# rubengooj/pl-slam

Hardware: AMD Instinct MI355X
Metric: stereo pairs/sec (1500 ORB + 200 LBD BF-match) (higher is better)
Workload: dtype fp4; 1 GPU; C2: synthetic 752x480 stereo stream, 1500 ORB + 200 LBD per image, ORB+LBD L<->R and prev<->curr, mutual + ratio (StVO::match), then StereoFrame's gates over the L<->R tables (config_kitti.yaml:25-...; mutual=True, distinct_batches_in_rotation=3, stereo_gates=True, kernel=k_scan_sym_mfma_i, mfma_form=0

## Files before the change

### plslam_amd/csrc/hamming_mfma_i.hip

```cpp
#include "mfma_h_common.hpp"

#include <type_traits>


namespace plslam {

namespace {
constexpr uint32_t MI_MAG = FP4_FOUR;
constexpr int MI_DSHIFT = 5;
constexpr uint32_t MI_ACC_BITS = 0x4B000000u + 4096u;
constexpr uint32_t MI_KEY16_MAX = 0x3FFFu;
constexpr uint32_t MI_COL_PENALTY = 0x4000u;
constexpr int MI_SCALE_A = 0, MI_SCALE_B = 0;
constexpr uint32_t MI_NONE16 = 0x7BFFu;
constexpr uint32_t MI_NONE32 = MI_NONE16 * 0x00010001u;
constexpr int MI_RESCAN_BATCH = 2;
constexpr int MI_RESCAN_BATCH16 = 2;
constexpr int MI_VGPRS = 168;
}

#ifdef PLSLAM_MI_PROF
constexpr int MI_PROF_WGS = 65536;
__device__ unsigned long long g_mi_prof[MI_PROF_WGS * 4];
#define PLSLAM_MI_TICK() __builtin_readcyclecounter()
#endif

template <bool DIRECTED>
__global__ void __launch_bounds__(256, 3) __attribute__((amdgpu_num_vgpr(MI_VGPRS / 2)))
k_scan_sym_mfma_i(const SymDesc* __restrict__ syms, const BlockDesc* __restrict__ blocks, int32_t* __restrict__ zero, int nzero, int nblocks)
{
    constexpr int ROWX_STRIDE = 33;
    constexpr int MI_ROW_STRIDE = MH_ROW_STRIDE, MI_TILE_BYTES = MH_TILE_N * MI_ROW_STRIDE;
    constexpr int PARK_OFF = 2 * MI_TILE_BYTES;
    constexpr int SMEM_BYTES = PARK_OFF + 4 * 16 * 64 * 8;
    static_assert(SMEM_BYTES >= 4 * 64 * ROWX_STRIDE * 4, "the transpose must fit");
    __shared__ __attribute__((aligned(16))) uint8_t smem[SMEM_BYTES];
    __shared__ __attribute__((aligned(16))) uint32_t colstage[MH_CGROUP * 256];
    constexpr int RING = 3;
    __shared__ __attribute__((aligned(16))) uint32_t rawring[RING][256];
    uint8_t* const btile = smem;
    u32x2_t* const park = reinterpret_cast<u32x2_t*>(smem + PARK_OFF) + (threadIdx.x >> 6) * (16 * 64) + (threadIdx.x & 63);

#ifdef PLSLAM_MI_PROF
    const unsigned long long prof_t0 = PLSLAM_MI_TICK();
    unsigned long long prof_loop = 0, prof_fin = 0, prof_tl = 0;
#endif
    if (blockIdx.x == 0)
        for (int i = threadIdx.x; i < nzero; i += 256) zero[i] = 0;
    asm volatile("s_setreg_imm32_b32 hwreg(HW_REG_MODE, 6, 2), 3");

    (void)nblocks;
    const int wg = xcd_remap_(blockIdx.x, gridDim.x);
    const BlockDesc bd = blocks[wg];
    if (bd.item < 0) return;
    const SymDesc sd = syms[bd.item];
    const int n1 = sd.n1, n2 = sd.n2;
    const MhLayout L(n2);
    const int ntiles = L.ntiles, nfull = L.nfull, rag_s = L.rag_s;
    const int n2p = (MH_TILE_N * ntiles + 255) & ~255;
    const int tid = threadIdx.x, lane = tid & 63;
    const int w = __builtin_amdgcn_readfirstlane(tid >> 6);
    const int c = lane & 31, g = lane >> 5;
    const gcu32_t araw = (gcu32_t) reinterpret_cast<const uint32_t*>(sd.a);
    const int iw = bd.row0 + 32 * w;

    i32x4 afrag[2][MH_KSTEPS];

    uint32_t gm[16];
#pragma unroll
    for (int s = 0; s < 16; ++s) gm[s] = MI_NONE32;

    u32x16 seed;
#pragma unroll
    for (int r = 0; r < 16; ++r) seed[r] = MI_ACC_BITS + (uint32_t)(16 * g + r);
    asm volatile("" : "+v"(seed));
    const int rest = n2 - (nfull >> 4) * MH_GROUP_ROWS;
    auto lane_lim = [&]() __attribute__((always_inline)) -> int {
        const int cc = (int)(threadIdx.x & 31u), v = rest - rag_s * cc;
        return rag_s == 0 ? 0 : (v < 0 ? 0 : (v > rag_s ? rag_s : v));
    };
    const int lim_part = rag_s ? rest % rag_s : 0;
    const int mask_from = rest - 31 * rag_s < 0 ? 0 : rest - 31 * rag_s;

    const bool block_ragged = bd.row0 + 256 > n1;
    const bool wide_part = !DIRECTED && (sd.flags & 1);
    const gu32_t part = DIRECTED ? (gu32_t) nullptr : (gu32_t) sd.part21 + (size_t)(bd.row0 >> 8) * n2p * (wide_part ? 2 : 1);
    uint32_t* const cstage = colstage + 64 * w;
#pragma unroll
    for (int k = 0; k < 2; ++k) *reinterpret_cast<i32x4*>(colstage + 8 * tid + 4 * k) = i32x4{-1, -1, -1, -1};

    const int ej = tid >> 3, ewd4 = (tid & 7) * 4;
    const PLSLAM_GLOBAL char* const bbytes = (const PLSLAM_GLOBAL char*) sd.b;
    auto load_raw = [&](int t) __attribute__((always_inline)) -> uint32_t {
        const int tc = t < ntiles ? t : ntiles - 1;
        const int gbase = (tc >> 4) * MH_GROUP_ROWS;
        const uint32_t s = tc < nfull ? (uint32_t)MH_GROUP : (uint32_t)rag_s;
        uint32_t row = __umul24((uint32_t)ej, s) + (uint32_t)(tc & 15);
        const uint32_t last = (uint32_t)(n2 - 1 - gbase);
        row = row < last ? row : last;
        return *reinterpret_cast<gcu32_t>(bbytes + (size_t)gbase * 32 + (row * 32u + (uint32_t)ewd4));
    };
    auto load_raw_async = [&](int t, uint32_t slot_b) __attribute__((always_inline)) {
        const int tc = t < ntiles ? t : ntiles - 1;
        const uint32_t s = tc < nfull ? (uint32_t)MH_GROUP : (uint32_t)rag_s;
        const uint32_t first = ((uint32_t)(tc & ~15) << 5) + (uint32_t)(tc & 15);
        uint32_t row = __umul24((uint32_t)ej, s) + first;
        const uint32_t last = (uint32_t)(n2 - 1);
        row = row < last ? row : last;
        const uint32_t voff = row * 32u + (uint32_t)ewd4;
        const uint32_t lds_dst = (uint32_t)(uintptr_t)(&rawring[0][64 * w]) + slot_b;
        asm volatile("s_mov_b32 m0, %2\n\ts_nop 0\n\tglobal_load_lds_dword %0, %1" : : "v"(voff), "s"(bbytes), "s"(lds_dst) : "memory", "m0");
    };
    uint32_t pf32 = 0;
    auto load_raw_async_full = [&](uint32_t slot_b) __attribute__((always_inline)) {
        const uint32_t voff = (uint32_t)(ej * (MH_GROUP * 32) + ewd4) + pf32;
        const uint32_t lds_dst = (uint32_t)(uintptr_t)(&rawring[0][64 * w]) + slot_b;
        asm volatile("s_mov_b32 m0, %2\n\ts_nop 0\n\tglobal_load_lds_dword %0, %1" : : "v"(voff), "s"(bbytes), "s"(lds_dst) : "memory", "m0");
    };
    auto take_raw = [&](uint32_t slot_b) __attribute__((always_inline)) -> uint32_t {
        asm volatile("s_waitcnt vmcnt(2)" ::: "memory");
        return *reinterpret_cast<const uint32_t*>(reinterpret_cast<const uint8_t*>(&rawring[0][0]) + slot_b + (ej * 32 + ewd4));
    };
    auto expand_store = [&](uint32_t raw, int buf, int tn, bool full = false) __attribute__((always_inline)) {
        uint8_t* dst = btile + buf * MI_TILE_BYTES + ej * MI_ROW_STRIDE + ewd4 * 4;
        i32x4 v = expand_dword_fp4<false, MI_MAG>(raw);
        if (!full && tn >= nfull && (tn & 15) >= mask_from) {
            const int vm = (int)(__umul24((uint32_t)rag_s, (uint32_t)ej) + (uint32_t)(tn & 15)) < rest ? -1 : 0;
            v &= i32x4{vm, vm, vm, vm};
        }
        *reinterpret_cast<i32x4*>(dst) = v;
    };

    int wt0 = 0, wt1 = ntiles < MH_WINDOW ? ntiles : MH_WINDOW;
    uint32_t ring_slot = 1024;

    const uint64_t part_u = (uint64_t)(uintptr_t)part;
    const uint64_t part_s = ((uint64_t)(uint32_t)__builtin_amdgcn_readfirstlane((int)(part_u >> 32)) << 32) |
                            (uint32_t)__builtin_amdgcn_readfirstlane((int)(uint32_t)part_u);
    auto combine_columns = [&](int kb) __attribute__((always_inline)) {
        if (DIRECTED) return;
        uint32_t l_;
        asm volatile("v_mbcnt_lo_u32_b32 %0, -1, 0\n\tv_mbcnt_hi_u32_b32 %0, -1, %0" : "=&v"(l_));
        const uint32_t* const src = colstage + 512 * w + (((l_ & 32u) << 3) | (l_ & 31u));
        uint32_t p[8];
#pragma unroll
        for (int v = 0; v < 4; ++v) { p[2 * v] = src[64 * v]; p[2 * v + 1] = src[64 * v + 32]; }
        if (block_ragged) {
#pragma unroll
            for (int q = 0; q < 8; ++q) {
                const int base = bd.row0 + 32 * (q >> 1) + 16 * (q & 1);
                const uint32_t strike = (base >= n1 ? MI_NONE16 : 0u) | (base + 128 >= n1 ? MI_NONE16 << 16 : 0u);
                p[q] = pk_max16(p[q], strike);
            }
        }
        auto pk_merge = [](uint32_t& a0, uint32_t& a1, uint32_t c0, uint32_t c1) {
            const uint32_t m = pk_max16(a0, c0);
            a0 = pk_min16(a0, c0);
            a1 = pk_min16(m, pk_min16(a1, c1));
        };
        uint32_t k0, k1;
        if (!wide_part) {
            uint32_t lo[4], hi[4], enc[4];
#pragma unroll
            for (int q = 0; q < 4; ++q) { lo[q] = pk_min16(p[2 * q], p[2 * q + 1]); hi[q] = pk_max16(p[2 * q], p[2 * q + 1]); }
#pragma unroll
            for (int q = 0; q < 4; ++q) {
                uint32_t t;
                asm("v_pk_add_u16 %0, %1, %2" : "=v"(t) : "v"(lo[q]), "v"((uint32_t)(32 * q) * 0x00010001u));
                asm("v_pk_mad_u16 %0, %1, %2, %3 clamp" : "=v"(enc[q]) : "v"(lo[q] & 0xFFE0FFE0u), "v"(0x00030003u), "v"(t));
            }
            const uint32_t best = pk_min16(pk_min16(enc[0], enc[1]), pk_min16(enc[2], enc[3]));
            pk_merge(lo[0], hi[0], lo[1], hi[1]);
            pk_merge(lo[2], hi[2], lo[3], hi[3]);
            pk_merge(lo[0], hi[0], lo[2], hi[2]);
            const uint32_t e0 = best & 0xFFFFu, u0 = best >> 16, e1 = hi[0] & 0xFFE0u, u1 = (hi[0] >> 16) & 0xFFE0u;
            k0 = e0 + (e0 & 0xFF80u);
            k1 = e1 << 3;
            merge2(k0, k1, u0 + (u0 & 0xFF80u) + 128u, u1 << 3);
        } else {
#pragma unroll
            for (int q = 0; q < 8; ++q) {
                const uint32_t t = p[q] & 0x001F001Fu;
                uint32_t sh;
                asm("v_pk_lshlrev_b16 %0, %1, %2" : "=v"(sh) : "v"(0x00020002u), "v"(p[q] & 0xFFE0FFE0u));
                p[q] = sh | t | ((uint32_t)(q >> 1) << 5) * 0x00010001u;
            }
            uint32_t lo[4], hi[4];
#pragma unroll
            for (int q = 0; q < 4; ++q) { lo[q] = pk_min16(p[2 * q], p[2 * q + 1]); hi[q] = pk_max16(p[2 * q], p[2 * q + 1]); }
            pk_merge(lo[0], hi[0], lo[1], hi[1]);
            pk_merge(lo[2], hi[2], lo[3], hi[3]);
            pk_merge(lo[0], hi[0], lo[2], hi[2]);
            const uint32_t e0 = lo[0] & 0xFFFFu, e1 = hi[0] & 0xFFFFu, u0 = lo[0] >> 16, u1 = hi[0] >> 16;
            k0 = e0 + (e0 & 0xFF80u); k1 = e1 + (e1 & 0xFF80u);
            merge2(k0, k1, u0 + (u0 & 0xFF80u) + 128u, u1 + (u1 & 0xFF80u) + 128u);
        }
        const uint32_t slot4 = (uint32_t)(256 * kb + 64 * w) * 4u;
        if (!wide_part) {
            const uint32_t e = (umin_(k0, 0x1FFFFu) << 9) | umin_(k1 >> 8, 511u);
            PLSLAM_GLOBAL uint32_t* dst = (PLSLAM_GLOBAL uint32_t*)((PLSLAM_GLOBAL char*)(uintptr_t)(part_s + slot4) + 4u * l_);
            __builtin_nontemporal_store(e, dst);
        } else {
            const u32x2_t e = {k0, k1};
            PLSLAM_GLOBAL u32x2_t* dst = (PLSLAM_GLOBAL u32x2_t*)((PLSLAM_GLOBAL char*)(uintptr_t)(part_s + 2u * slot4) + 8u * l_);
            __builtin_nontemporal_store(e, dst);
        }
    };
    auto push_groups = [&gm, &wt0, &park](int t, auto final_tag, u32x2_t* rb) __attribute__((always_inline)) {
        constexpr bool FINAL = decltype(final_tag)::value;
        const uint32_t grp = (uint32_t)(((t - wt0) >> 4) & 3);
        const uint32_t gtag = grp * 0x00010001u;
        uint32_t gtv = gtag;
        asm volatile("" : "+v"(gtv));
        auto retag = [&](uint32_t x) -> uint32_t {
            uint32_t r;
            asm("v_and_or_b32 %0, %1, %2, %3" : "=v"(r) : "v"(x), "s"(0xFFE0FFE0u), "v"(gtv));
            return r;
        };
        if (grp == 0) {
#pragma unroll
            for (int s = 0; s < 16; ++s) {
// ... 85 lines not shown
            }
            finish_columns(t - 1, cm0_prev, cm1);
            if (U == 0 && ((t - 1) & (MH_GROUP - 1)) == MH_GROUP - 1) push_groups(t - 1, std::false_type{}, nullptr);
        }
        __builtin_amdgcn_sched_barrier(0);
        asm volatile("v_mfma_f32_32x32x64_f8f6f4 %0, %1, %2, %3 cbsz:4 blgp:4" : "=&v"(m1) : "v"(afrag[1][0]), "v"(bfr[0]), "v"(cseed));
        __builtin_amdgcn_sched_barrier(0);
        PLSLAM_MI_EPI2(m0, 0, 0)
        PLSLAM_MI_MMA(m1, 1, 1, m1)    PLSLAM_MI_EPI2(m0, 0, 2)
        PLSLAM_MI_MMA(m1, 1, 2, m1)    PLSLAM_MI_EPI2(m0, 0, 4)
        PLSLAM_MI_MMA(m1, 1, 3, m1)    PLSLAM_MI_EPI2(m0, 0, 6)
        cm0_prev = cf_join();
    };
    auto epilogue = [&](int t) __attribute__((always_inline)) {
        float cfa = 0.0f;
        asm volatile("s_nop 7\n\ts_nop 7");
        __builtin_amdgcn_sched_barrier(0);
        PLSLAM_MI_EPI2(m1, 1, 0) PLSLAM_MI_EPI2(m1, 1, 2) PLSLAM_MI_EPI2(m1, 1, 4) PLSLAM_MI_EPI2(m1, 1, 6)
        finish_columns(t, cm0_prev, __builtin_bit_cast(uint32_t, cfa));
    };
    auto pipeline = [&](u32x2_t* rb) __attribute__((always_inline)) {
        {
            u32x16 none;
#pragma unroll
            for (int r = 0; r < 16; ++r) asm volatile("v_mov_b32 %0, %1" : "=v"(none[r]) : "s"(MI_NONE32));
            m1 = __builtin_bit_cast(f32x16, none);
        }
        int tb = wt0;
        {
            const int lim = (wt1 < nfull ? wt1 : nfull) - 7;
            pf32 = (((uint32_t)((tb + 4) & ~15) << 5) + (uint32_t)((tb + 4) & 15)) * 32u;
            for (; tb < lim; tb += 4) {
                tile_step(tb, std::integral_constant<int, 0>{}, tb != wt0, std::true_type{});
                tile_step(tb + 1, std::integral_constant<int, 1>{}, true, std::true_type{});
                tile_step(tb + 2, std::integral_constant<int, 2>{}, true, std::true_type{});
                tile_step(tb + 3, std::integral_constant<int, 3>{}, true, std::true_type{});
            }
        }
        for (; tb < wt1; tb += 4) {
            tile_step(tb, std::integral_constant<int, 0>{}, tb != wt0, std::false_type{});
            if (tb + 1 < wt1) tile_step(tb + 1, std::integral_constant<int, 1>{}, true, std::false_type{});
            if (tb + 2 < wt1) tile_step(tb + 2, std::integral_constant<int, 2>{}, true, std::false_type{});
            if (tb + 3 < wt1) tile_step(tb + 3, std::integral_constant<int, 3>{}, true, std::false_type{});
        }
        if (!DIRECTED && ((wt1 - 1) & (MH_CGROUP - 1)) == 0 && wt1 - 9 >= wt0) {
            __syncthreads();
            combine_columns((wt1 - 9) >> 3);
            __syncthreads();
        }
        epilogue(wt1 - 1);
        push_groups(wt1 - 1, std::true_type{}, rb);
    };
#undef PLSLAM_MI_EPI2
#undef PLSLAM_MI_MMA
#undef PLSLAM_MI_READ_B

    auto finish_rows = [&](const u32x2_t* rb) __attribute__((always_inline)) {
        uint32_t* rowx = reinterpret_cast<uint32_t*>(smem) + w * (64 * ROWX_STRIDE);
#pragma unroll
        for (int s = 0; s < 16; ++s) {
            const int lrow = 32 * (s >> 3) + 16 * g + (s & 7);
            rowx[lrow * ROWX_STRIDE + c] = __builtin_amdgcn_perm(rb[s].y, rb[s].x, 0x05040100u);
            rowx[(lrow + 8) * ROWX_STRIDE + c] = __builtin_amdgcn_perm(rb[s].y, rb[s].x, 0x07060302u);
        }
        __builtin_amdgcn_fence(__ATOMIC_RELEASE, "wavefront");
        __builtin_amdgcn_wave_barrier();
        __builtin_amdgcn_fence(__ATOMIC_ACQUIRE, "wavefront");
        uint32_t k0 = 0xFFFFFFFFu, k1 = 0xFFFFFFFFu;
        const uint32_t* mine = rowx + lane * ROWX_STRIDE;
#pragma unroll
        for (int cls = 0; cls < 32; ++cls) {
            uint32_t x;
            asm("v_lshl_or_b32 %0, %1, 16, %2" : "=v"(x) : "v"(mine[cls]), "n"(cls));
            asm("v_med3_u32 %0, %1, %2, %0" : "+v"(k1) : "v"(k0), "v"(x));
            k0 = umin_(k0, x);
        }
        {
            const uint32_t cs = k0 & 31u;
            k1 = umin_(k1, (mine[cs] & 0xFFFF0000u) | cs);
        }
        int row = iw + lane + (lane & 32) * 3;
        asm volatile("" : "+v"(row));
        if (row < n1) {
            const gu2_t out = (gu2_t) reinterpret_cast<u32x2_t*>(sd.keys12) + row;
            const gcu32x4_t ap = (gcu32x4_t)(araw + (size_t)row * 8);
            const u32x4_t a_lo = ap[0], a_hi = ap[1];
            auto group_of = [&](uint32_t k, uint32_t& jbase, uint32_t& cnt) {
                const uint32_t t0 = (uint32_t)wt0 + (((k >> 16) & 3u) << 4);
                const uint32_t s = t0 < (uint32_t)nfull ? (uint32_t)MH_GROUP : (uint32_t)rag_s;
                jbase = (t0 >> 4) * MH_GROUP_ROWS + s * (k & 0xFFFFu);
                cnt = s;
            };
            auto rescan = [&](uint32_t jbase, uint32_t cnt, uint32_t& best, uint32_t& second) {
                best = second = KEY_NONE;
                const uint32_t left = (uint32_t)n2 - jbase;
                const uint32_t nvalid = cnt < left ? cnt : left;
                const PLSLAM_GLOBAL char* const rbp = bbytes + (size_t)jbase * 32;
#pragma unroll
                for (int k0_ = 0; k0_ < MH_GROUP; k0_ += MI_RESCAN_BATCH) {
                    u32x4_t bl[MI_RESCAN_BATCH], bh[MI_RESCAN_BATCH];
#pragma unroll
                    for (int q = 0; q < MI_RESCAN_BATCH; ++q) {
                        const uint32_t kk = (uint32_t)(k0_ + q) < nvalid ? (uint32_t)(k0_ + q) : nvalid - 1u;
                        const gcu32x4_t bp = (gcu32x4_t)(rbp + kk * 32u);
                        bl[q] = bp[0];
                        bh[q] = bp[1];
                    }
#pragma unroll
                    for (int q = 0; q < MI_RESCAN_BATCH; ++q) {
                        const uint32_t d = hamming256(a_lo, a_hi, bl[q], bh[q]);
                        const uint32_t cand = (uint32_t)(k0_ + q) < nvalid ? ((d << KEY_IDX_BITS) | (jbase + (uint32_t)(k0_ + q))) : KEY_NONE;
                        second = umin_(second, umax_(best, cand));
                        best = umin_(best, cand);
                    }
                }
            };
            auto rescan16 = [&](uint32_t jb, uint32_t& best, uint32_t& second) {
                uint32_t bk = 0xFFFFFFFFu, sk = 0xFFFFFFFFu;
                const PLSLAM_GLOBAL char* const rbp = bbytes + (size_t)jb * 32;
                constexpr int RB = MI_RESCAN_BATCH16;
#pragma unroll
                for (int k0_ = 0; k0_ < 16; k0_ += RB) {
                    u32x4_t bl[RB], bh[RB];
#pragma unroll
                    for (int q = 0; q < RB; ++q) {
                        const gcu32x4_t bp = (gcu32x4_t)(rbp + (k0_ + q) * 32);
                        bl[q] = bp[0];
                        bh[q] = bp[1];
                    }
#pragma unroll
                    for (int q = 0; q < RB; ++q) {
                        const uint32_t d = hamming256(a_lo, a_hi, bl[q], bh[q]);
                        uint32_t x;
                        asm("v_lshl_or_b32 %0, %1, 4, %2" : "=v"(x) : "v"(d), "n"(k0_ + q));
                        asm("v_med3_u32 %0, %1, %2, %0" : "+v"(sk) : "v"(bk), "v"(x));
                        bk = umin_(bk, x);
                    }
                }
                best = ((bk >> 4) << KEY_IDX_BITS) | (jb + (bk & 15u));
                second = ((sk >> 4) << KEY_IDX_BITS) | (jb + (sk & 15u));
            };
            uint32_t r0 = KEY_NONE, r1 = KEY_NONE;
            if ((k0 >> 16) <= MI_KEY16_MAX) {
                uint32_t jb, cnt, in2;
                group_of(k0, jb, cnt);
                const uint32_t jsh = jb + 16u <= (uint32_t)n2 ? jb : (uint32_t)n2 - 16u;
                const bool guarded = n2 < 16 || jsh < (uint32_t)wt0 * MH_TILE_N;
                if (__builtin_amdgcn_ballot_w64(guarded) == 0) rescan16(jsh, r0, in2);
                else rescan(jb, cnt, r0, in2);
                if ((k1 >> 16) <= MI_KEY16_MAX) {
                    uint32_t jb1, cnt1;
                    group_of(k1, jb1, cnt1);
                    uint32_t o1 = ((k1 >> (16 + MI_DSHIFT)) << KEY_IDX_BITS) | jb1;
                    if ((sd.flags & 1) && (o1 >> KEY_IDX_BITS) <= (in2 >> KEY_IDX_BITS)) {
                        uint32_t b1, s1;
                        rescan(jb1, cnt1, b1, s1);
                        o1 = b1;
                    }
                    r1 = umin_(in2, o1);
                } else {
                    r1 = in2;
                }
            }
            if (wt0 > 0) {
                const u32x2_t prev = *out;
                merge2(r0, r1, prev.x, prev.y);
            }
            *out = u32x2_t{r0, r1};
        }
        __builtin_amdgcn_fence(__ATOMIC_RELEASE, "wavefront");
        __builtin_amdgcn_wave_barrier();
    };

    uint32_t raw_first = load_raw(0);
    load_raw_async(1, 1024);
    load_raw_async(2, 2048);
    load_raw_async(3, 0);
#pragma unroll
    for (int mt = 0; mt < 2; ++mt) {
        const int row = bd.row0 + 128 * mt + 32 * w + 16 * ((c >> 2) & 1) + (c & 3) + 4 * (c >> 3);
        const int rrow = row < n1 ? row : n1 - 1;
        const gcu32_t p = araw + (size_t)rrow * 8 + g;
#pragma unroll
        for (int ks = 0; ks < MH_KSTEPS; ++ks) afrag[mt][ks] = expand_dword_fp4<true, MI_MAG>(p[2 * ks]);
    }

#ifdef PLSLAM_MI_PROF
    const unsigned long long prof_t1 = PLSLAM_MI_TICK();
#endif
    for (;;) {
#ifdef PLSLAM_MI_PROF
        prof_tl = PLSLAM_MI_TICK();
#endif
        expand_store(raw_first, 0, wt0);
        ring_slot = 1024;
        u32x2_t rb[16];
        __builtin_amdgcn_s_setprio(1);
        pipeline(rb);
        __builtin_amdgcn_s_setprio(0);
#ifdef PLSLAM_MI_PROF
        { const unsigned long long t = PLSLAM_MI_TICK(); prof_loop += t - prof_tl; prof_tl = t; }
#endif
        __syncthreads();
        combine_columns((wt1 - 1) >> 3);
        finish_rows(rb);
#ifdef PLSLAM_MI_PROF
        prof_fin += PLSLAM_MI_TICK() - prof_tl;
#endif
        if (wt1 == ntiles) break;
        __syncthreads();
        wt0 = wt1;
        wt1 = ntiles < wt0 + MH_WINDOW ? ntiles : wt0 + MH_WINDOW;
        raw_first = load_raw(wt0);
        load_raw_async(wt0 + 1, 1024);
        load_raw_async(wt0 + 2, 2048);
        load_raw_async(wt0 + 3, 0);
    }
#ifdef PLSLAM_MI_PROF
    if (threadIdx.x == 0 && blockIdx.x < MI_PROF_WGS) {
        g_mi_prof[4 * blockIdx.x + 0] = prof_t1 - prof_t0;
        g_mi_prof[4 * blockIdx.x + 1] = prof_loop;
        g_mi_prof[4 * blockIdx.x + 2] = prof_fin;
        g_mi_prof[4 * blockIdx.x + 3] = ((unsigned long long)ntiles << 40) | (PLSLAM_MI_TICK() - prof_t0);
    }
#endif
}

#ifdef PLSLAM_MI_PROF
extern "C" int plslam_debug_k1i_profile(unsigned long long* out, int nwg)
{
    if (nwg > MI_PROF_WGS) nwg = MI_PROF_WGS;
    return hipMemcpyFromSymbol(out, HIP_SYMBOL(g_mi_prof), sizeof(unsigned long long) * 4 * (size_t)nwg) == hipSuccess ? nwg : -1;
}
#endif

int launch_scan_sym_mfma_i(const SymDesc* d_sym, const BlockDesc* d_blocks, int nblocks, int32_t* d_zero, int nzero,
                           bool directed, hipStream_t s)
{
    if (nblocks <= 0) return PLSLAM_OK;
    if (directed) hipLaunchKernelGGL((k_scan_sym_mfma_i<true>), dim3(nblocks), dim3(256), 0, s, d_sym, d_blocks, d_zero, nzero, nblocks);
    else hipLaunchKernelGGL((k_scan_sym_mfma_i<false>), dim3(nblocks), dim3(256), 0, s, d_sym, d_blocks, d_zero, nzero, nblocks);
    PLSLAM_HIP_CHECK(hipGetLastError());
    return PLSLAM_OK;
}

}
```

### plslam_amd/csrc/match_planner.hpp

```cpp
#pragma once

#include <algorithm>
#include <vector>

#include "match_tables.hpp"

namespace plslam {

struct PlanOptions {
    int cu_count = 0;
    int scan_variant = PLSLAM_SCAN_AUTO, scan_block = 0, sym_rows = 0, group_cap = 0, mfma_form = 0, col_split = 0, exact_second = 0;
    int split_target = 0, split_min_tiles = 0, split_post = 0, post_xcd = 2, post_fuse = 0, fuse = 0;
    int rows_wpq = 0, rows_lpq = 0;
    int sym_block_rows[2] = {0, 0};
    int sym_partial_rows[2] = {0, 0};
    int merge16_cols[3] = {0, 0, 0};
    int fix16_cols[3] = {0, 0, 0};

    bool takes_device_row_count() const
    {
        return (scan_variant == PLSLAM_SCAN_AUTO || scan_variant == PLSLAM_SCAN_MFMA) && (mfma_form == 0 || mfma_form == 2) &&
               col_split != 1 && split_post != 1 && fuse != 2;
    }
};

enum class ProblemPath : int32_t {
    empty,
    scan,
    sym,
    directed,
    split,
};

struct ProblemPlan {
    ProblemPath path;
    int32_t nsplit, cstep;
    int64_t key_row, part_row, tmp_row;
};

struct PlanChoice {
    PlanOptions opts;
    const char* error = nullptr;
    bool small = false;
    int scan_variant = 0, block_threads = 0;
    int rows_scan = 0;
    bool sym_mfma = false;
    bool dpair = false;
    int mfma_form = 0;
    int sym_rows = 1;
    int rows_sym = 0, rows_partial = 0;
    bool fused = false;
    bool col_split = false;
    bool split_post = false;
    bool exact_second = false;
    int merge_parts = 1;
    int merge_cols = 0;
    size_t group_cap = 2;
    int64_t key_rows = 0, part_rows = 0, tmp_rows = 0;
    bool counts_in_place = false, scatter_counts = false;
    std::vector<ProblemPlan> per;

    bool h_tables() const { return sym_mfma && mfma_form_is_h(mfma_form) && !fused; }
    bool partials16() const { return sym_mfma && mfma_form != 1; }
    bool lazy_keys() const { return h_tables() && !exact_second; }
    int64_t part_units(int32_t n1, int32_t n2) const
    {
        if (h_tables()) return (int64_t)((n1 + 255) / 256) * ((n2 + 255) / 256) * (exact_second ? 256 : 128);
        return (int64_t)((n1 + 63) / 64) * ((n2 + 255) / 256) * 128;
    }
};

#define PLSLAM_PLAN_REQUIRE(cond, code)   \
    do {                                  \
        if (!(cond)) {                    \
            c.error = #cond;              \
            return (code);                \
        }                                 \
    } while (0)

inline int plan_decide(const PlanOptions& o, const plslam_match_problem* probs, int32_t nprob, bool has_n1_dev0, PlanChoice& c)
{
    c.error = nullptr;
    c.per.clear();
    c.opts = o;
    PLSLAM_PLAN_REQUIRE(nprob >= 0, PLSLAM_EINVAL);
// ... 52 lines not shown
        for (int32_t i = 0; i < nprob; ++i)
            if (is_sym(probs[i])) { cols += probs[i].n2; max_nwb = std::max(max_nwb, (probs[i].n1 + 63) / 64); }
        const int64_t lanes = 64 * 4 * (int64_t)o.cu_count * 4;
        c.merge_parts = (max_nwb >= 64 && cols * 16 <= lanes) ? 16 : (max_nwb >= 32 && cols * 4 <= lanes) ? 4 : 1;
    }
    const int parts_k = c.merge_parts >= 16 ? 2 : c.merge_parts >= 4 ? 1 : 0;
    c.merge_cols = c.h_tables() ? o.fix16_cols[parts_k] : o.merge16_cols[parts_k];
    c.scan_variant = use_wpq ? PLSLAM_SCAN_WAVE_PER_QUERY : PLSLAM_SCAN_LANE_PER_QUERY;
    c.block_threads = use_wpq ? 256 : (o.scan_block ? o.scan_block : 256);
    c.rows_scan = use_wpq ? o.rows_wpq : o.rows_lpq;
    c.group_cap = o.group_cap > 0 ? (size_t)o.group_cap : (c.sym_rows == 4 ? 8 : 2);

    const int64_t want = c.col_split ? ((o.split_target > 0 ? o.split_target : 3) * (int64_t)o.cu_count + mf_row_blocks - 1) / mf_row_blocks : 1;
    const int32_t min_tiles = o.split_min_tiles > 0 ? o.split_min_tiles : 4;
    c.split_post = c.col_split && !c.h_tables() && !c.fused && o.split_post != 1 && nprob > 0;
    c.key_rows = c.part_rows = c.tmp_rows = 0;
    c.counts_in_place = nprob > 0;
    bool any_counter = false;
    for (int32_t i = 0; i < nprob; ++i) {
        const plslam_match_problem& p = probs[i];
        PLSLAM_PLAN_REQUIRE(p.n1 >= 0 && p.n2 >= 0, PLSLAM_EINVAL);
        PLSLAM_PLAN_REQUIRE(p.n1 == 0 || p.d1 != nullptr, PLSLAM_EINVAL);
        PLSLAM_PLAN_REQUIRE(p.n2 == 0 || p.d2 != nullptr, PLSLAM_EINVAL);
        PLSLAM_PLAN_REQUIRE(p.n1 == 0 || p.matches_12 != nullptr, PLSLAM_EINVAL);
        PLSLAM_PLAN_REQUIRE((reinterpret_cast<uintptr_t>(p.d1) & 3) == 0, PLSLAM_EINVAL);
        PLSLAM_PLAN_REQUIRE((reinterpret_cast<uintptr_t>(p.d2) & 3) == 0, PLSLAM_EINVAL);
        PLSLAM_PLAN_REQUIRE(p.n2 <= PLSLAM_MAX_TRAIN_ROWS, PLSLAM_ERANGE);
        PLSLAM_PLAN_REQUIRE(!p.mutual || p.n1 <= PLSLAM_MAX_TRAIN_ROWS, PLSLAM_ERANGE);
        ProblemPlan q{ProblemPath::empty, 1, 0, c.key_rows, c.part_rows, c.tmp_rows};
        const bool both = p.n1 > 0 && p.n2 > 0;
        if (c.col_split && both) {
            const int32_t tiles = (p.n2 + 31) / 32;
            const int32_t per = std::max((int32_t)((tiles + want - 1) / want), min_tiles);
            const int32_t ns = (tiles + per - 1) / per;
            if (ns > 1) { q.nsplit = ns; q.cstep = per * 32; }
        }
        q.path = q.nsplit > 1 ? ProblemPath::split : is_sym(p) ? ProblemPath::sym : c.sym_mfma && both ? ProblemPath::directed
                 : p.n1 > 0 ? ProblemPath::scan : ProblemPath::empty;
        c.key_rows += p.n1 + (p.mutual ? p.n2 : 0);
        if (q.path == ProblemPath::split) {
            for (int32_t s = 0; p.mutual && s < q.nsplit; ++s) c.part_rows += c.part_units(p.n1, std::min(q.cstep, p.n2 - s * q.cstep));
            c.tmp_rows += (int64_t)q.nsplit * p.n1;
        } else if (q.path == ProblemPath::sym) {
            c.part_rows += c.partials16() ? c.part_units(p.n1, p.n2) : (int64_t)((p.n1 + c.rows_partial - 1) / c.rows_partial) * p.n2;
        }
        c.split_post = c.split_post && is_sym(p) && !p.keep_prior;
        any_counter = any_counter || p.n_matches != nullptr;
        c.counts_in_place = c.counts_in_place && p.n_matches != nullptr && p.n_matches == probs[0].n_matches + i;
        c.per.push_back(q);
    }
    c.scatter_counts = any_counter && !c.counts_in_place;
    PLSLAM_PLAN_REQUIRE(c.key_rows < (int64_t(1) << 31), PLSLAM_ERANGE);
    if (has_n1_dev0 && !c.split_post) return PLSLAM_ENOTSUP;
    return PLSLAM_OK;
}
#undef PLSLAM_PLAN_REQUIRE

struct PlanBases {
    uint32_t* keys = nullptr;
    uint32_t* partials = nullptr;
    uint32_t* rowtmp = nullptr;
    int32_t* counts = nullptr;
    const int32_t* n1_dev0 = nullptr;
};

struct PlanTables {
    std::vector<ScanDesc> scans;
    std::vector<int32_t> scan_problem;
    std::vector<SymDesc> syms, dirs;
    std::vector<ProblemDesc> probs;
    std::vector<BlockDesc> scan_blocks, sym_blocks, dir_blocks, merge_blocks, fin_blocks;
    std::vector<int32_t*> user_counts;
    bool sym_mfma_multi = false, dir_multi = false;
    bool post_fused = false;
    size_t post_lds = 0;
    int32_t fin_row = 0;
    plslam_plan_info info{};
    enum { SCANS, SYMS, PROBS, SCAN_BLOCKS, SYM_BLOCKS, MERGE_BLOCKS, FIN_BLOCKS, COUNT_DST, DIRS, DIR_BLOCKS, NPIECES };
    struct Piece { const void* src; size_t bytes, off; } piece[NPIECES] = {};
    size_t total = 0;
    struct Group { int64_t cost; int32_t first, count; size_t xcd, at; };
    std::vector<Group> groups;
    std::vector<BlockDesc> dealt;
};

template <class KeyOf, class CostOf>
inline size_t deal_to_xcds(PlanTables& t, std::vector<BlockDesc>& blocks, size_t cap, KeyOf key_of, CostOf cost_of)
{
    t.groups.clear();
    for (size_t i = 0; i < blocks.size();) {
        size_t j = i;
        while (j < blocks.size() && j - i < cap && key_of(blocks[j]) == key_of(blocks[i])) ++j;
        t.groups.push_back({cost_of(blocks[i]), (int32_t)i, (int32_t)(j - i), 0, 0});
        i = j;
    }
    std::stable_sort(t.groups.begin(), t.groups.end(), [](const PlanTables::Group& a, const PlanTables::Group& b) { return a.cost > b.cost; });
    size_t len[8] = {0, 0, 0, 0, 0, 0, 0, 0}, x = 0;
    for (PlanTables::Group& g : t.groups) {
        size_t best = x;
        for (size_t k = 0; k < 8; ++k) {
            const size_t cand = (x + k) & 7;
            if (len[cand] < len[best]) best = cand;
        }
        g.xcd = best;
        g.at = len[best];
        len[best] += (size_t)g.count;
        x = (best + 1) & 7;
    }
    const size_t L = *std::max_element(len, len + 8);
    t.dealt.assign(8 * L, BlockDesc{-1, 0});
    for (const PlanTables::Group& g : t.groups)
        for (int32_t k = 0; k < g.count; ++k) t.dealt[g.xcd * L + g.at + (size_t)k] = blocks[(size_t)g.first + k];
    blocks.swap(t.dealt);
    return L;
}

inline void plan_tables(const PlanChoice& c, const plslam_match_problem* probs, const PlanBases& b, PlanTables& t)
{
    const int32_t nprob = (int32_t)c.per.size();
    t.scans.clear(); t.scan_problem.clear(); t.syms.clear(); t.dirs.clear(); t.probs.clear(); t.user_counts.clear();
    t.scan_blocks.clear(); t.sym_blocks.clear(); t.dir_blocks.clear(); t.merge_blocks.clear(); t.fin_blocks.clear();
    t.sym_mfma_multi = t.dir_multi = false;
    int64_t evals = 0, devals = 0, abytes = 0;
    auto blocks_of = [](std::vector<BlockDesc>& tab, size_t item, int32_t n, int32_t step) {
        for (int32_t r0 = 0; r0 < n; r0 += step) tab.push_back({(int32_t)item, r0});
    };
    for (int32_t i = 0; i < nprob; ++i) {
        const plslam_match_problem& p = probs[i];
        const ProblemPlan& q = c.per[(size_t)i];
        ProblemDesc pd{};
        pd.n1 = p.n1; pd.n2 = p.n2; pd.nnr = p.nnr; pd.mutual = p.mutual ? 1 : 0;
        pd.keep_prior = p.keep_prior ? 1 : 0;
        pd.matches_12 = p.matches_12;
        pd.n_matches = b.counts + i;
        t.user_counts.push_back(p.n_matches);
        uint32_t* k12 = b.keys + 2 * q.key_row;
        uint32_t* k21 = p.mutual ? k12 + 2 * (int64_t)p.n1 : nullptr;
        pd.keys12 = k12;
        pd.keys21 = k21;
        pd.d1 = p.d1; pd.d2 = p.d2;
        pd.gate = -1;
        const int64_t nn = (int64_t)p.n1 * p.n2;
        const bool on_mfma = q.path == ProblemPath::split || (c.sym_mfma && (q.path == ProblemPath::sym || q.path == ProblemPath::directed));
        if (!(c.fused && on_mfma)) blocks_of(t.fin_blocks, (size_t)i, p.n1, 256);
        SymDesc y{};
        y.flags = c.exact_second ? 1 : 0;
        switch (q.path) {
        case ProblemPath::split: {
            uint32_t* tmp = b.rowtmp + 2 * q.tmp_row;
            pd.split_tmp = tmp; pd.keys12_out = k12; pd.nsplit = q.nsplit; pd.cstep = q.cstep;
            pd.lazy21 = p.mutual && c.lazy_keys();
            std::vector<SymDesc>& dst = p.mutual ? t.syms : t.dirs;
            int64_t part_row = q.part_row;
            for (int32_t s = 0; s < q.nsplit; ++s) {
                const int32_t c0 = s * q.cstep, n2s = std::min(q.cstep, p.n2 - c0);
                y.a = p.d1; y.b = p.d2 + (size_t)c0 * 32;
                y.keys12 = tmp + 2 * (int64_t)s * p.n1;
                y.n1 = p.n1; y.n2 = n2s;
                if (c.split_post) { y.mutual = i + 1; y.matches_12 = s == 0 ? p.matches_12 : nullptr; y.n1_dev = b.n1_dev0; }
                if (p.mutual) {
                    y.keys21 = k21 + 2 * (size_t)c0;
                    y.part21 = b.partials + 2 * part_row;
                    y.n_iblk = (p.n1 + c.rows_partial - 1) / c.rows_partial;
                    part_row += c.part_units(p.n1, n2s);
                    blocks_of(t.merge_blocks, dst.size(), (n2s + 31) & ~31, c.merge_cols);
                }
                blocks_of(p.mutual ? t.sym_blocks : t.dir_blocks, dst.size(), p.n1, 256);
                if (n2s > 2048) (p.mutual ? t.sym_mfma_multi : t.dir_multi) = true;
                dst.push_back(y);
            }
            evals += nn;
            devals += (p.mutual ? 2 : 1) * nn;
            abytes += p.mutual ? 2 * 32LL * (p.n1 + p.n2) + 16LL * (p.n1 + p.n2) : 32LL * (p.n1 + p.n2) + 16LL * p.n1;
            break;
        }
        case ProblemPath::sym:
            pd.lazy21 = c.lazy_keys();
            y.a = p.d1; y.b = p.d2; y.keys12 = k12; y.keys21 = k21;
            y.part21 = b.partials + 2 * q.part_row;
            pd.part21 = y.part21;
            y.n1 = p.n1; y.n2 = p.n2; y.n_iblk = (p.n1 + c.rows_partial - 1) / c.rows_partial;
            if (c.split_post) { y.mutual = i + 1; y.matches_12 = p.matches_12; y.n1_dev = b.n1_dev0; }
            if (c.fused) {
                y.mutual = 1; y.matches_12 = p.matches_12; y.n_matches = pd.n_matches; y.nnr = p.nnr;
                t.sym_blocks.push_back({(int32_t)t.syms.size(), 0});
            } else {
                blocks_of(t.sym_blocks, t.syms.size(), p.n1, c.rows_sym);
                if (c.partials16()) blocks_of(t.merge_blocks, t.syms.size(), (p.n2 + 31) & ~31, c.merge_cols);
                else blocks_of(t.merge_blocks, t.syms.size(), p.n2, 256);
            }
            if (c.sym_mfma && p.n2 > 2048) t.sym_mfma_multi = true;
            t.syms.push_back(y);
            evals += nn;
            devals += 2 * nn;
            abytes += 2 * 32LL * (p.n1 + p.n2) + 16LL * (p.n1 + p.n2);
            break;
        case ProblemPath::directed:
            for (int dir = 0; dir < (p.mutual ? 2 : 1); ++dir) {
                y.a = dir ? p.d2 : p.d1; y.b = dir ? p.d1 : p.d2; y.keys12 = dir ? k21 : k12;
                y.n1 = dir ? p.n2 : p.n1; y.n2 = dir ? p.n1 : p.n2;
                if (c.fused && !p.mutual) {
                    y.mutual = 0; y.matches_12 = p.matches_12; y.n_matches = pd.n_matches; y.nnr = p.nnr;
                    t.dir_blocks.push_back({(int32_t)t.dirs.size(), 0});
                } else {
                    blocks_of(t.dir_blocks, t.dirs.size(), y.n1, 256);
                }
                if (y.n2 > 2048) t.dir_multi = true;
                t.dirs.push_back(y);
                evals += nn;
                devals += nn;
                abytes += 32LL * (p.n1 + p.n2) + 16LL * y.n1;
            }
            break;
        case ProblemPath::scan:
            for (int dir = 0; dir < (p.mutual && p.n2 > 0 ? 2 : 1); ++dir) {
                const ScanDesc sc = dir ? ScanDesc{p.d2, p.d1, k21, p.n2, p.n1} : ScanDesc{p.d1, p.d2, k12, p.n1, p.n2};
                blocks_of(t.scan_blocks, t.scans.size(), sc.nq, c.rows_scan);
                t.scans.push_back(sc);
                t.scan_problem.push_back(i);
                evals += nn;
                devals += nn;
                abytes += 32LL * (p.n1 + p.n2) + 16LL * sc.nq;
            }
            break;
        case ProblemPath::empty:
            break;
        }
        t.probs.push_back(pd);
    }
    auto item_of = [](const BlockDesc& e) { return e.item; };
    auto stream_cost = [&c](const std::vector<SymDesc>& d) {
        return [&c, &d](const BlockDesc& e) { return (int64_t)d[(size_t)e.item].n2 * (c.fused ? d[(size_t)e.item].n1 : 1); };
    };
    if (!t.sym_blocks.empty()) deal_to_xcds(t, t.sym_blocks, c.group_cap, item_of, stream_cost(t.syms));
    if (!t.dir_blocks.empty()) deal_to_xcds(t, t.dir_blocks, c.group_cap, item_of, stream_cost(t.dirs));
    if (c.scan_variant != PLSLAM_SCAN_WAVE_PER_QUERY && !t.scan_blocks.empty())
        deal_to_xcds(t, t.scan_blocks, c.group_cap, [&t](const BlockDesc& e) { return t.scan_problem[(size_t)e.item]; },
                     [&t](const BlockDesc& e) { return (int64_t)t.scans[(size_t)e.item].nt; });
    t.fin_row = 0;
    if (c.opts.post_xcd == 2 && t.fin_blocks.size() >= 64)
        t.fin_row = (int32_t)deal_to_xcds(t, t.fin_blocks, (size_t)-1, item_of, [](const BlockDesc&) { return (int64_t)0; });

    bool pf = c.opts.post_fuse == 2 && c.lazy_keys() && !c.col_split && nprob > 0;
    int32_t max_n2 = 0;
    for (int32_t i = 0; pf && i < nprob; ++i) {
        pf = c.per[(size_t)i].path == ProblemPath::sym && t.probs[(size_t)i].part21 != nullptr && probs[i].n2 <= POST_FUSED_MAX_N2 &&
             (probs[i].n1 + 255) / 256 <= POST_FUSED_MAX_ROW_BLOCKS;
        max_n2 = std::max(max_n2, probs[i].n2);
    }
    t.post_fused = pf;
    t.post_lds = pf ? sizeof(uint32_t) * 2 * (size_t)((max_n2 + 63) & ~63) : 0;

    const int32_t nsym = (int32_t)t.syms.size(), ndir = (int32_t)t.dirs.size();
    t.info.distance_evals = evals;
    t.info.directed_evals = devals;
    t.info.algorithmic_bytes = abytes;
    t.info.n_scans = (int32_t)t.scans.size() + 2 * nsym + ndir;
    t.info.scan_blocks = (int32_t)(t.scan_blocks.size() + t.sym_blocks.size() + t.dir_blocks.size());
    t.info.scan_variant = nsym ? (c.sym_mfma ? PLSLAM_SCAN_MFMA : PLSLAM_SCAN_SYMMETRIC) : (ndir ? PLSLAM_SCAN_MFMA : c.scan_variant);
    t.info.scan_block_threads = nsym ? (c.sym_rows == 4 && !c.sym_mfma ? 64 : 256) : (ndir ? 256 : c.block_threads);

    auto put = [&t](int k, const auto& v, size_t n) { t.piece[k] = {v.data(), n * sizeof(v[0]), 0}; };
    put(PlanTables::SCANS, t.scans, t.scans.size());
    put(PlanTables::SYMS, t.syms, t.syms.size());
    put(PlanTables::PROBS, t.probs, t.probs.size());
    put(PlanTables::SCAN_BLOCKS, t.scan_blocks, t.scan_blocks.size());
    put(PlanTables::SYM_BLOCKS, t.sym_blocks, t.sym_blocks.size());
    put(PlanTables::MERGE_BLOCKS, t.merge_blocks, t.merge_blocks.size());
    put(PlanTables::FIN_BLOCKS, t.fin_blocks, t.fin_blocks.size());
    put(PlanTables::COUNT_DST, t.user_counts, c.scatter_counts ? t.user_counts.size() : 0);
    put(PlanTables::DIRS, t.dirs, t.dirs.size());
    put(PlanTables::DIR_BLOCKS, t.dir_blocks, t.dir_blocks.size());
    t.total = 0;
    for (PlanTables::Piece& x : t.piece) { x.off = t.total; t.total += align256(x.bytes); }
    if (t.total == 0) t.total = 256;
}

}
```

### plslam_amd/csrc/match_tables.hpp

```cpp
#pragma once

#include <stddef.h>
#include <stdint.h>

#include "plslam_hip.h"

namespace plslam {

struct ScanDesc {
    const uint8_t* q;
    const uint8_t* t;
    uint32_t* keys;
    int32_t nq, nt;
};

struct ProblemDesc {
    const uint32_t* keys12;
    const uint32_t* keys21;
    int32_t* matches_12;
    int32_t* n_matches;
    int32_t n1, n2;
    float nnr;
    int32_t mutual;
    const uint32_t* split_tmp;
    uint32_t* keys12_out;
    int32_t nsplit, cstep;
    int32_t keep_prior;
    int32_t lazy21;
    const uint8_t* d1;
    const uint8_t* d2;
    int32_t gate, pad2;
    const uint32_t* part21;
    int16_t* matches_16;
};

struct BlockDesc {
    int32_t item;
    int32_t row0;
};

struct SymDesc {
    const uint8_t* a;
    const uint8_t* b;
    uint32_t* keys12;
    uint32_t* keys21;
    uint32_t* part21;
    int32_t n1, n2;
    int32_t n_iblk;
    int32_t mutual;
    int32_t* matches_12;
    int32_t* n_matches;
    float nnr;
    int32_t flags;
    const int32_t* n1_dev;
};

constexpr size_t align256(size_t bytes) { return (bytes + 255) & ~size_t(255); }
struct Carver {
    size_t off = 0;
    size_t take(size_t bytes) { const size_t o = off; off += align256(bytes); return o; }
};

static_assert(sizeof(ScanDesc) == 32, "ScanDesc layout");
static_assert(sizeof(SymDesc) == 88, "SymDesc layout");
static_assert(sizeof(ProblemDesc) == 120, "ProblemDesc layout");
static_assert(sizeof(BlockDesc) == 8, "BlockDesc layout");

constexpr int POST_FUSED_MAX_N2 = 4096;
constexpr int POST_FUSED_MAX_ROW_BLOCKS = 16;
constexpr int PLSLAM_K1F_FUSED_MAX_N2 = 4096;

inline bool mfma_form_is_h(int form) { return form == 0 || form == 4 || form == 5; }
#ifndef PLSLAM_BUILD_LEGACY_SCANS
#define PLSLAM_BUILD_LEGACY_SCANS 0
#endif
inline bool mfma_form_built(int form) { return PLSLAM_BUILD_LEGACY_SCANS || form == 0 || form == 2 || form == 5; }

}
```

Measured before the change: 1.627 million stereo pairs/s.

## Pair sibling problems sharing the same query set into one workgroup pass

The planner links two symmetric problems that share the same A descriptors and row count (for example left vs right and left vs previous) when both have a small B set. The second problem then gets no blocks of its own. Each workgroup keeps its A fragments resident and streams the sibling's B set after finishing the first, resetting its per-problem state in between. This is meant to cut workgroup count, duplicate A loads and per-block prologue cost. In exchange each workgroup runs longer, SymDesc grows, and the XCD dealing cost now counts both problems.

Result: no change. 1.643 million stereo pairs/s (median of 6 runs) (+1.0%).

```diff
diff --git a/plslam_amd/csrc/hamming_mfma_i.hip b/plslam_amd/csrc/hamming_mfma_i.hip
--- a/plslam_amd/csrc/hamming_mfma_i.hip
+++ b/plslam_amd/csrc/hamming_mfma_i.hip
@@ -17,6 +17,7 @@
 constexpr int MI_RESCAN_BATCH = 2;
 constexpr int MI_RESCAN_BATCH16 = 2;
 constexpr int MI_VGPRS = 168;
+static_assert(K1I_SIBLING_MAX_N2 == MH_WINDOW * MH_TILE_N, "a sibling is one window of b long");
 }
 
 #ifdef PLSLAM_MI_PROF
@@ -43,7 +44,7 @@
 
 #ifdef PLSLAM_MI_PROF
     const unsigned long long prof_t0 = PLSLAM_MI_TICK();
-    unsigned long long prof_loop = 0, prof_fin = 0, prof_tl = 0;
+    unsigned long long prof_loop = 0, prof_fin = 0, prof_tl = 0, prof_pro = 0, prof_tiles = 0;
 #endif
     if (blockIdx.x == 0)
         for (int i = threadIdx.x; i < nzero; i += 256) zero[i] = 0;
@@ -54,10 +55,15 @@
     const BlockDesc bd = blocks[wg];
     if (bd.item < 0) return;
     const SymDesc sd = syms[bd.item];
-    const int n1 = sd.n1, n2 = sd.n2;
-    const MhLayout L(n2);
-    const int ntiles = L.ntiles, nfull = L.nfull, rag_s = L.rag_s;
-    const int n2p = (MH_TILE_N * ntiles + 255) & ~255;
+    const int sib = DIRECTED ? -1 : sd.next;
+    const SymDesc* const sdn = syms + (sib < 0 ? bd.item : sib);
+    const uint8_t* const sib_b = sdn->b;
+    uint32_t* const sib_keys12 = sdn->keys12;
+    uint32_t* const sib_part21 = sdn->part21;
+    const int sib_n2 = sdn->n2;
+    const int n1 = sd.n1;
+    int n2, ntiles, nfull, rag_s;
+    int n2p;
     const int tid = threadIdx.x, lane = tid & 63;
     const int w = __builtin_amdgcn_readfirstlane(tid >> 6);
     const int c = lane & 31, g = lane >> 5;
@@ -71,26 +77,49 @@
     for (int s = 0; s < 16; ++s) gm[s] = MI_NONE32;
 
     u32x16 seed;
-#pragma unroll
-    for (int r = 0; r < 16; ++r) seed[r] = MI_ACC_BITS + (uint32_t)(16 * g + r);
-    asm volatile("" : "+v"(seed));
-    const int rest = n2 - (nfull >> 4) * MH_GROUP_ROWS;
+    auto reset_seed = [&]() __attribute__((always_inline)) {
+#pragma unroll
+        for (int r = 0; r < 16; ++r) seed[r] = MI_ACC_BITS + (uint32_t)(16 * g + r);
+        asm volatile("" : "+v"(seed));
+    };
+    reset_seed();
+    int rest;
     auto lane_lim = [&]() __attribute__((always_inline)) -> int {
         const int cc = (int)(threadIdx.x & 31u), v = rest - rag_s * cc;
         return rag_s == 0 ? 0 : (v < 0 ? 0 : (v > rag_s ? rag_s : v));
     };
-    const int lim_part = rag_s ? rest % rag_s : 0;
-    const int mask_from = rest - 31 * rag_s < 0 ? 0 : rest - 31 * rag_s;
+    int lim_part;
+    int mask_from;
 
     const bool block_ragged = bd.row0 + 256 > n1;
     const bool wide_part = !DIRECTED && (sd.flags & 1);
-    const gu32_t part = DIRECTED ? (gu32_t) nullptr : (gu32_t) sd.part21 + (size_t)(bd.row0 >> 8) * n2p * (wide_part ? 2 : 1);
     uint32_t* const cstage = colstage + 64 * w;
-#pragma unroll
-    for (int k = 0; k < 2; ++k) *reinterpret_cast<i32x4*>(colstage + 8 * tid + 4 * k) = i32x4{-1, -1, -1, -1};
+    auto clear_colstage = [&]() __attribute__((always_inline)) {
+#pragma unroll
+        for (int k = 0; k < 2; ++k) *reinterpret_cast<i32x4*>(colstage + 8 * tid + 4 * k) = i32x4{-1, -1, -1, -1};
+    };
+    clear_colstage();
 
     const int ej = tid >> 3, ewd4 = (tid & 7) * 4;
-    const PLSLAM_GLOBAL char* const bbytes = (const PLSLAM_GLOBAL char*) sd.b;
+    const PLSLAM_GLOBAL char* bbytes;
+    uint32_t* keys12;
+    uint64_t part_s = 0;
+    auto set_problem = [&](const uint8_t* b_, uint32_t* keys12_, uint32_t* part21_, int n2_) __attribute__((always_inline)) {
+        const MhLayout L(n2_);
+        n2 = n2_; ntiles = L.ntiles; nfull = L.nfull; rag_s = L.rag_s;
+        n2p = (MH_TILE_N * ntiles + 255) & ~255;
+        rest = n2 - (nfull >> 4) * MH_GROUP_ROWS;
+        lim_part = rag_s ? rest % rag_s : 0;
+        mask_from = rest - 31 * rag_s < 0 ? 0 : rest - 31 * rag_s;
+        bbytes = (const PLSLAM_GLOBAL char*) b_;
+        keys12 = keys12_;
+        if (!DIRECTED) {
+            const uint64_t part_u = (uint64_t)(uintptr_t)((gu32_t) part21_ + (size_t)(bd.row0 >> 8) * n2p * (wide_part ? 2 : 1));
+            part_s = ((uint64_t)(uint32_t)__builtin_amdgcn_readfirstlane((int)(part_u >> 32)) << 32) |
+                     (uint32_t)__builtin_amdgcn_readfirstlane((int)(uint32_t)part_u);
+        }
+    };
+    set_problem(sd.b, sd.keys12, sd.part21, sd.n2);
     auto load_raw = [&](int t) __attribute__((always_inline)) -> uint32_t {
         const int tc = t < ntiles ? t : ntiles - 1;
         const int gbase = (tc >> 4) * MH_GROUP_ROWS;
@@ -132,11 +161,9 @@
     };
 
     int wt0 = 0, wt1 = ntiles < MH_WINDOW ? ntiles : MH_WINDOW;
+    bool sib_left = sib >= 0;
     uint32_t ring_slot = 1024;
 
-    const uint64_t part_u = (uint64_t)(uintptr_t)part;
-    const uint64_t part_s = ((uint64_t)(uint32_t)__builtin_amdgcn_readfirstlane((int)(part_u >> 32)) << 32) |
-                            (uint32_t)__builtin_amdgcn_readfirstlane((int)(uint32_t)part_u);
     auto combine_columns = [&](int kb) __attribute__((always_inline)) {
         if (DIRECTED) return;
         uint32_t l_;
@@ -388,7 +415,7 @@
         int row = iw + lane + (lane & 32) * 3;
         asm volatile("" : "+v"(row));
         if (row < n1) {
-            const gu2_t out = (gu2_t) reinterpret_cast<u32x2_t*>(sd.keys12) + row;
+            const gu2_t out = (gu2_t) reinterpret_cast<u32x2_t*>(keys12) + row;
             const gcu32x4_t ap = (gcu32x4_t)(araw + (size_t)row * 8);
             const u32x4_t a_lo = ap[0], a_hi = ap[1];
             auto group_of = [&](uint32_t k, uint32_t& jbase, uint32_t& cnt) {
@@ -513,7 +540,34 @@
 #ifdef PLSLAM_MI_PROF
         prof_fin += PLSLAM_MI_TICK() - prof_tl;
 #endif
-        if (wt1 == ntiles) break;
+        if (wt1 == ntiles) {
+            if (DIRECTED || !sib_left) break;
+            sib_left = false;
+#ifdef PLSLAM_MI_PROF
+            const unsigned long long prof_s0 = PLSLAM_MI_TICK();
+            prof_tiles += (unsigned long long)ntiles;
+#endif
+            __syncthreads();
+            {
+                uint64_t b_ = (uint64_t)(uintptr_t)sib_b;
+                int n2_ = sib_n2;
+                asm volatile("" : "+s"(b_), "+s"(n2_));
+                set_problem(reinterpret_cast<const uint8_t*>((uintptr_t)b_), sib_keys12, sib_part21, n2_);
+            }
+            wt0 = 0;
+            wt1 = ntiles;
+            raw_first = load_raw(0);
+            load_raw_async(1, 1024);
+            load_raw_async(2, 2048);
+            load_raw_async(3, 0);
+            clear_colstage();
+            reset_seed();
+            cm0_prev = MI_NONE32;
+#ifdef PLSLAM_MI_PROF
+            prof_pro += PLSLAM_MI_TICK() - prof_s0;
+#endif
+            continue;
+        }
         __syncthreads();
         wt0 = wt1;
         wt1 = ntiles < wt0 + MH_WINDOW ? ntiles : wt0 + MH_WINDOW;
@@ -524,10 +578,10 @@
     }
 #ifdef PLSLAM_MI_PROF
     if (threadIdx.x == 0 && blockIdx.x < MI_PROF_WGS) {
-        g_mi_prof[4 * blockIdx.x + 0] = prof_t1 - prof_t0;
+        g_mi_prof[4 * blockIdx.x + 0] = prof_t1 - prof_t0 + prof_pro;
         g_mi_prof[4 * blockIdx.x + 1] = prof_loop;
         g_mi_prof[4 * blockIdx.x + 2] = prof_fin;
-        g_mi_prof[4 * blockIdx.x + 3] = ((unsigned long long)ntiles << 40) | (PLSLAM_MI_TICK() - prof_t0);
+        g_mi_prof[4 * blockIdx.x + 3] = ((prof_tiles + (unsigned long long)ntiles) << 40) | (PLSLAM_MI_TICK() - prof_t0);
     }
 #endif
 }
diff --git a/plslam_amd/csrc/match_planner.hpp b/plslam_amd/csrc/match_planner.hpp
--- a/plslam_amd/csrc/match_planner.hpp
+++ b/plslam_amd/csrc/match_planner.hpp
@@ -1,6 +1,8 @@
 #pragma once
 
 #include <algorithm>
+#include <map>
+#include <utility>
 #include <vector>
 
 #include "match_tables.hpp"
@@ -219,6 +221,7 @@
     struct Group { int64_t cost; int32_t first, count; size_t xcd, at; };
     std::vector<Group> groups;
     std::vector<BlockDesc> dealt;
+    std::map<std::pair<const uint8_t*, int32_t>, int32_t> open_heads;
 };
 
 template <class KeyOf, class CostOf>
@@ -258,6 +261,8 @@
     t.scans.clear(); t.scan_problem.clear(); t.syms.clear(); t.dirs.clear(); t.probs.clear(); t.user_counts.clear();
     t.scan_blocks.clear(); t.sym_blocks.clear(); t.dir_blocks.clear(); t.merge_blocks.clear(); t.fin_blocks.clear();
     t.sym_mfma_multi = t.dir_multi = false;
+    t.open_heads.clear();
+    const bool pair_siblings = c.h_tables() && mfma_form_is_i(c.mfma_form) && !c.fused && !c.split_post;
     int64_t evals = 0, devals = 0, abytes = 0;
     auto blocks_of = [](std::vector<BlockDesc>& tab, size_t item, int32_t n, int32_t step) {
         for (int32_t r0 = 0; r0 < n; r0 += step) tab.push_back({(int32_t)item, r0});
@@ -322,7 +327,16 @@
                 y.mutual = 1; y.matches_12 = p.matches_12; y.n_matches = pd.n_matches; y.nnr = p.nnr;
                 t.sym_blocks.push_back({(int32_t)t.syms.size(), 0});
             } else {
-                blocks_of(t.sym_blocks, t.syms.size(), p.n1, c.rows_sym);
+                bool is_sibling = false;
+                if (pair_siblings && p.n2 <= K1I_SIBLING_MAX_N2) {
+                    const auto slot = t.open_heads.emplace(std::make_pair(p.d1, p.n1), (int32_t)t.syms.size());
+                    if (!slot.second) {
+                        t.syms[(size_t)slot.first->second].next = (int32_t)t.syms.size();
+                        t.open_heads.erase(slot.first);
+                        is_sibling = true;
+                    }
+                }
+                if (!is_sibling) blocks_of(t.sym_blocks, t.syms.size(), p.n1, c.rows_sym);
                 if (c.partials16()) blocks_of(t.merge_blocks, t.syms.size(), (p.n2 + 31) & ~31, c.merge_cols);
                 else blocks_of(t.merge_blocks, t.syms.size(), p.n2, 256);
             }
@@ -367,7 +381,10 @@
     }
     auto item_of = [](const BlockDesc& e) { return e.item; };
     auto stream_cost = [&c](const std::vector<SymDesc>& d) {
-        return [&c, &d](const BlockDesc& e) { return (int64_t)d[(size_t)e.item].n2 * (c.fused ? d[(size_t)e.item].n1 : 1); };
+        return [&c, &d](const BlockDesc& e) {
+            const SymDesc& y = d[(size_t)e.item];
+            return (int64_t)y.n2 * (c.fused ? y.n1 : 1) + (y.next >= 0 ? d[(size_t)y.next].n2 : 0);
+        };
     };
     if (!t.sym_blocks.empty()) deal_to_xcds(t, t.sym_blocks, c.group_cap, item_of, stream_cost(t.syms));
     if (!t.dir_blocks.empty()) deal_to_xcds(t, t.dir_blocks, c.group_cap, item_of, stream_cost(t.dirs));
diff --git a/plslam_amd/csrc/match_tables.hpp b/plslam_amd/csrc/match_tables.hpp
--- a/plslam_amd/csrc/match_tables.hpp
+++ b/plslam_amd/csrc/match_tables.hpp
@@ -53,6 +53,7 @@
     float nnr;
     int32_t flags;
     const int32_t* n1_dev;
+    int32_t next = -1;
 };
 
 constexpr size_t align256(size_t bytes) { return (bytes + 255) & ~size_t(255); }
@@ -62,7 +63,7 @@
 };
 
 static_assert(sizeof(ScanDesc) == 32, "ScanDesc layout");
-static_assert(sizeof(SymDesc) == 88, "SymDesc layout");
+static_assert(sizeof(SymDesc) == 96, "SymDesc layout");
 static_assert(sizeof(ProblemDesc) == 120, "ProblemDesc layout");
 static_assert(sizeof(BlockDesc) == 8, "BlockDesc layout");
 
@@ -71,6 +72,8 @@
 constexpr int PLSLAM_K1F_FUSED_MAX_N2 = 4096;
 
 inline bool mfma_form_is_h(int form) { return form == 0 || form == 4 || form == 5; }
+inline bool mfma_form_is_i(int form) { return form == 0 || form == 5; }
+constexpr int K1I_SIBLING_MAX_N2 = 2048;
 #ifndef PLSLAM_BUILD_LEGACY_SCANS
 #define PLSLAM_BUILD_LEGACY_SCANS 0
 #endif
```
